# Murmeldyret/cubesat-APDS

Measured on AMD Instinct MI355X. Metric: frames/sec (detect+match+homography) 4k×4k tile vs 1M-desc DB; Mmatches/sec, higher is better.
Workload: dtype fp4 e2m1 operands / f32 accumulate = exact integer Hamming (match), f32 (AKAZE), f64 (homography solve)

## Files before the change

cubesat-apds_amd/csrc/common.h:

```cpp
#pragma once
#include <hip/hip_runtime.h>

#include <atomic>
#include <cstdint>
#include <cstdio>
#include <map>
#include <string>
#include <vector>

#include "../../include/apds.h"

#ifndef APDS_STAGE_WAVE_PRIO
#define APDS_STAGE_WAVE_PRIO 1
#endif
#define APDS_RAISE_WAVE_PRIORITY() __builtin_amdgcn_s_setprio(APDS_STAGE_WAVE_PRIO)

namespace apds {

struct Error {
    int code;
    std::string msg;
};

void set_last_error(const std::string& m);

[[noreturn]] inline void fail(int code, const std::string& m) { throw Error{code, m}; }

inline void hip_check(hipError_t e, const char* what, const char* file, int line) {
    if (e == hipSuccess) return;
    int code = APDS_ERR_INTERNAL;
    if (e == hipErrorNoDevice || e == hipErrorInvalidDevice || e == hipErrorNoBinaryForGpu || e == hipErrorInsufficientDriver ||
        e == hipErrorNotInitialized)
        code = APDS_ERR_NO_DEVICE;
    if (e == hipErrorOutOfMemory) code = APDS_ERR_NOMEM;
    char buf[512];
    snprintf(buf, sizeof buf, "%s failed: %s (%s:%d)", what, hipGetErrorString(e), file, line);
    (void)hipGetLastError();
    throw Error{code, buf};
}
#define HIP_CHECK(x) ::apds::hip_check((x), #x, __FILE__, __LINE__)
#define APDS_REQUIRE(cond, code, msg) \
    do {                               \
        if (!(cond)) ::apds::fail((code), (msg)); \
    } while (0)

struct ThreadCtx {
    int device = 0;
    bool ready = false;
    hipStream_t stream = nullptr;
    std::vector<std::pair<char*, size_t>> slabs;
    size_t slab_used = 0;
    size_t call_bytes = 0;
    bool timing = false;
    struct Ev {
        hipEvent_t a, b;
        hipStream_t s;
    };
    std::map<std::string, std::vector<Ev>> events;
    hipStream_t side = nullptr;
    std::vector<hipEvent_t> fork_events;
    hipEvent_t join_event = nullptr;
    int akaze_first_batch[2] = {8, 8};
    int akaze_batch_streak[2] = {0, 0};
    bool fork_open = false;
    int akaze_kp_estimate = 0;
    int* host_ints = nullptr;
    size_t host_ints_cap = 0;
    int* pinned_ints(size_t n);
    hipStream_t side_stream();
    hipStream_t side_pool[4] = {nullptr, nullptr, nullptr, nullptr};
    hipStream_t side_probe_caller = nullptr, side_probe_choice = nullptr;
    void drop_side();
    hipEvent_t fork_event(size_t i);

    hipEvent_t tail_event = nullptr, count_event = nullptr;
    hipStream_t tail_stream = nullptr;
    bool tail_pending = false;
    void mark_tail(hipStream_t s);
    void mark_tail_noexcept(hipStream_t s) noexcept;

    void ensure();
    void* alloc(size_t bytes);
    void ws_reset(hipStream_t for_stream = nullptr);
    template <class T>
    T* alloc_n(size_t n) { return static_cast<T*>(alloc(n * sizeof(T))); }
};
ThreadCtx& ctx();
std::atomic<int>& live_contexts();

hipStream_t side_stream_beside(hipStream_t caller);
bool take_cached_side_stream(int device, hipStream_t& out);
void cache_side_stream(int device, hipStream_t st);
unsigned stream_event_flags();

inline hipStream_t pick_stream(void* s) { return s ? static_cast<hipStream_t>(s) : ctx().stream; }

struct QueuedWorkspaceCall {
    ThreadCtx& c;
    hipStream_t s;
    explicit QueuedWorkspaceCall(hipStream_t st) : c(ctx()), s(st) { c.ws_reset(s); }
    ~QueuedWorkspaceCall() { c.mark_tail_noexcept(s); }
    QueuedWorkspaceCall(const QueuedWorkspaceCall&) = delete;
    QueuedWorkspaceCall& operator=(const QueuedWorkspaceCall&) = delete;
};

struct KernelTimer {
    ThreadCtx::Ev ev{};
    bool on;
    const char* name;
    KernelTimer(const char* nm, hipStream_t s) : on(ctx().timing), name(nm) {
        if (!on) return;
        ev.s = s;
        HIP_CHECK(hipEventCreate(&ev.a));
        HIP_CHECK(hipEventCreate(&ev.b));
        HIP_CHECK(hipEventRecord(ev.a, s));
    }
    ~KernelTimer() {
        if (!on) return;
        (void)hipEventRecord(ev.b, ev.s);
        ctx().events[name].push_back(ev);
    }
};

struct TraceRange {
    explicit TraceRange(const char* name);
    ~TraceRange();
    TraceRange(const TraceRange&) = delete;
    TraceRange& operator=(const TraceRange&) = delete;
};
#define APDS_RANGE(name) ::apds::TraceRange apds_trace_range_(name)

template <class F>
int guarded(F&& f) {
    try {
        f();
        return APDS_OK;
    } catch (const Error& e) {
        set_last_error(e.msg);
        return e.code;
    } catch (const std::bad_alloc&) {
        set_last_error("host allocation failed");
        return APDS_ERR_NOMEM;
    } catch (const std::exception& e) {
        set_last_error(e.what());
        return APDS_ERR_INTERNAL;
    } catch (...) {
        set_last_error("unknown failure");
        return APDS_ERR_INTERNAL;
    }
}

// ... 12 lines not shown
```

cubesat-apds_amd/csrc/config.h:

```cpp
#pragma once

namespace apds {

struct Config {
    int nld_strip;
    int sf_strip;
    int base_strip;
    int level_strip;
    int level_fuse;
    int level_stream;
    int level_stream_rows;
    int doh_strip;
    int doh_strip_rows;
    int kp_ranked;
    int kp_xcd;
    int half_fuse;
    int fed_shrink;
    int akaze_fork;
    int side_probe;
    int match_mfma;
    int match_mfma_kmax;
    int early_count;
    int l2_prio;
    int match_mfma_lds_pad;
    int match_mfma_prio;
    int match_mfma_sample;
    int match_mfma_splits;
    int match_mfma_xcd;
    int event_scope;
    int debug_host_time;
    int match_lds_cap;
    int match_sample;
    int ransac_batch;
    int pnp_batch;
    int l2_sample_div;
    int pipe_extract_workers;
    int pipe_match_split;
    int pipe_adaptive_cap;
    int pipe_prio;
    int loopback_lag_rank, loopback_lag_ms;
};

const Config& config();

}
```

cubesat-apds_amd/csrc/hamming_mfma.hip:

```cpp
#include <atomic>
#include <memory>

#include "config.h"
#include "kernels.h"
#include "topk_keys.h"

namespace apds {

typedef int hm_v8i __attribute__((ext_vector_type(8)));
typedef float hm_f32x4 __attribute__((ext_vector_type(4)));
typedef uint32_t hm_u32x4 __attribute__((ext_vector_type(4)));

#ifndef APDS_HM_WAVES
#define APDS_HM_WAVES 8
#endif
static constexpr int HM_WAVES = APDS_HM_WAVES;
static constexpr int HM_TM = 16 * HM_WAVES;
#ifndef APDS_HM_WPE
#define APDS_HM_WPE 4
#endif
#ifndef APDS_HM_TOP2_VGPRS
#define APDS_HM_TOP2_VGPRS (APDS_HM_WPE == 4 ? 104 : 512 / APDS_HM_WPE / 8 * 8)
#endif
static_assert(APDS_HM_TOP2_VGPRS % 8 == 0 && APDS_HM_WPE * APDS_HM_TOP2_VGPRS <= 512, "the cap is whole granules that fit the SIMD's file");
// ... 204 lines not shown
__device__ __forceinline__ void hm_load_queries(const uint4* query_fp4, const float* qpc, int nq, int q0, int col, int kq, uint4 (&B)[NC][4], float (&qq)[NC]) {
#pragma unroll
    for (int c = 0; c < NC; c++) {
        const int qi = min(q0 + 16 * c + col, nq - 1);
#pragma unroll
        for (int s = 0; s < 4; s++) B[c][s] = query_fp4[(size_t)qi * 16 + 4 * s + kq];
        qq[c] = qpc[qi];
    }
}
template <bool THR>
__device__ __forceinline__ uint32_t hm_start_value(const uint32_t* thr, int qi) {
    return THR ? thr[qi] : 0x7F800000u;
}
__device__ __forceinline__ uint32_t hm_distance(float qq, uint32_t d) { return (uint32_t)((int)(qq + __uint_as_float(d)) - HM_BIAS); }

template <int PRIO, bool THR>
__global__ __launch_bounds__(64 * HM_WAVES) __attribute__((amdgpu_waves_per_eu(APDS_HM_WPE, APDS_HM_WPE), amdgpu_num_vgpr(APDS_HM_TOP2_VGPRS / 2))) void hamming_mfma_kernel(const uint4* __restrict__ train_fp4, const float* __restrict__ tpc, int n_train,
                                                           const uint4* __restrict__ query_fp4, const float* __restrict__ qpc, int nq, int tiles_per_split,
                                                           int q_tiles, int splits, uint32_t index_base, const uint32_t* __restrict__ thr,
                                                           uint64_t* __restrict__ out) {
    const HmItem w = hm_work_item<HM_NC>(n_train, tiles_per_split, q_tiles, splits);
    const int split = w.split, q0 = w.q0, tile_begin = w.tile_begin, tile_end = w.tile_end, col = w.col, kq = w.kq;
    uint4 B[HM_NC][4];
    hm_load_operands<HM_NC>(query_fp4, nq, q0, col, kq, B);
    HmTop2 best[HM_NC];
#pragma unroll
    for (int c = 0; c < HM_NC; c++) {
        best[c].d0 = hm_start_value<THR>(thr, min(q0 + 16 * c + col, nq - 1));
        hm_settle(best[c].d0);
        best[c].d1 = best[c].d0;
        best[c].i0 = best[c].i1 = 0xFFFFFFFFu;
    }

    if (tile_begin < tile_end) {
        hm_scan_tiles<HM_NC, PRIO>(train_fp4, tpc, tile_begin, tile_end, B, index_base, [&](const hm_f32x4 (&a)[HM_NC], uint32_t row0) {
            bool hit[HM_NC];
#pragma unroll
            for (int c = 0; c < HM_NC; c++) {
                const uint32_t mn = min(min(__float_as_uint(a[c][0]), __float_as_uint(a[c][1])), min(__float_as_uint(a[c][2]), __float_as_uint(a[c][3])));
                hit[c] = mn < best[c].d1;
            }
#pragma unroll
            for (int c = 0; c < HM_NC; c++)
                if (__any(hit[c])) {
#pragma unroll
                    for (int j = 0; j < 4; j++) hm_insert(best[c], __float_as_uint(a[c][j]), row0 + j);
                }
        });
    }
#pragma unroll
    for (int c = 0; c < HM_NC; c++) {
        HmTop2 b = best[c];
#pragma unroll
        for (int off = 16; off < 64; off <<= 1) {
            const uint32_t od0 = (uint32_t)__shfl_xor((int)b.d0, off), od1 = (uint32_t)__shfl_xor((int)b.d1, off);
            const uint32_t oi0 = (uint32_t)__shfl_xor((int)b.i0, off), oi1 = (uint32_t)__shfl_xor((int)b.i1, off);
            HmTop2 m = b;
            auto ins = [&](uint32_t d, uint32_t i) {
                if (i == 0xFFFFFFFFu) return;
                if (d < m.d0 || (d == m.d0 && i < m.i0)) {
                    m.d1 = m.d0;
                    m.i1 = m.i0;
                    m.d0 = d;
                    m.i0 = i;
                } else if ((d < m.d1 || (d == m.d1 && i < m.i1)) && i != m.i0) {
                    m.d1 = d;
                    m.i1 = i;
                }
            };
            ins(od0, oi0);
            ins(od1, oi1);
            b = m;
        }
        const int qi = q0 + 16 * c + col;
        if (kq == 0 && qi < nq) {
            uint64_t* o = out + ((size_t)split * nq + qi) * 2;
            const float qq = qpc[qi];
            o[0] = b.i0 == 0xFFFFFFFFu ? EMPTY_KEY : make_key(hm_distance(qq, b.d0), b.i0);
            o[1] = b.i1 == 0xFFFFFFFFu ? EMPTY_KEY : make_key(hm_distance(qq, b.d1), b.i1);
        }
    }
}

template <int K>
struct HmTopK {
    uint32_t d[K];
    uint32_t i[K];
};
template <int K>
__device__ __forceinline__ void hm_insert_k(HmTopK<K>& b, uint32_t d, uint32_t idx) {
#pragma unroll
    for (int j = K - 1; j > 0; j--) {
        const bool shift = d < b.d[j - 1], here = d < b.d[j];
        b.i[j] = shift ? b.i[j - 1] : (here ? idx : b.i[j]);
        b.d[j] = shift ? b.d[j - 1] : (here ? d : b.d[j]);
    }
    const bool first = d < b.d[0];
    b.i[0] = first ? idx : b.i[0];
    b.d[0] = first ? d : b.d[0];
}
__device__ __forceinline__ uint64_t hm_shfl_xor_u64(uint64_t v, int off) {
    return ((uint64_t)(uint32_t)__shfl_xor((int)(uint32_t)(v >> 32), off) << 32) | (uint32_t)__shfl_xor((int)(uint32_t)v, off);
}

#ifndef APDS_HM_NC_K4
#define APDS_HM_NC_K4 2
#endif
#ifndef APDS_HM_NC_K8
#define APDS_HM_NC_K8 2
#endif
template <int K>
struct HmShape {
    static constexpr int NC = K <= 4 ? APDS_HM_NC_K4 : APDS_HM_NC_K8;
    static constexpr int Q = HM_WAVES * 16 * NC;
};

template <int K, int NC, int PRIO, bool THR>
__global__ __launch_bounds__(64 * HM_WAVES) __attribute__((amdgpu_waves_per_eu(APDS_HM_WPE, APDS_HM_WPE))) void hamming_mfma_topk_kernel(
    const uint4* __restrict__ train_fp4, const float* __restrict__ tpc, int n_train, const uint4* __restrict__ query_fp4, const float* __restrict__ qpc, int nq,
    int tiles_per_split, int q_tiles, int splits, uint32_t index_base, const uint32_t* __restrict__ thr, uint64_t* __restrict__ out) {
    const HmItem w = hm_work_item<NC>(n_train, tiles_per_split, q_tiles, splits);
    const int split = w.split, q0 = w.q0, tile_begin = w.tile_begin, tile_end = w.tile_end, col = w.col, kq = w.kq;
    uint4 B[NC][4];
    float qq[NC];
    hm_load_queries<NC>(query_fp4, qpc, nq, q0, col, kq, B, qq);
    HmTopK<K> best[NC];
#pragma unroll
    for (int c = 0; c < NC; c++) {
        uint32_t start = hm_start_value<THR>(thr, min(q0 + 16 * c + col, nq - 1));
        hm_settle(start), hm_settle(qq[c]);
#pragma unroll
        for (int j = 0; j < K; j++) best[c].d[j] = start, best[c].i[j] = 0xFFFFFFFFu;
    }

    if (tile_begin < tile_end) {
        hm_scan_tiles<NC, PRIO>(train_fp4, tpc, tile_begin, tile_end, B, index_base, [&](const hm_f32x4 (&a)[NC], uint32_t row0) {
            bool hit[NC];
#pragma unroll
            for (int c = 0; c < NC; c++) {
                const uint32_t mn = min(min(__float_as_uint(a[c][0]), __float_as_uint(a[c][1])), min(__float_as_uint(a[c][2]), __float_as_uint(a[c][3])));
                hit[c] = mn < best[c].d[K - 1];
            }
#pragma unroll
            for (int c = 0; c < NC; c++)
                if (__any(hit[c])) {
#pragma unroll
                    for (int j = 0; j < 4; j++) {
                        const uint32_t v = __float_as_uint(a[c][j]);
                        if (__any(v < best[c].d[K - 1])) hm_insert_k<K>(best[c], v, row0 + j);
                    }
                }
        });
    }
#pragma unroll
    for (int c = 0; c < NC; c++) {
        uint64_t key[K];
#pragma unroll
        for (int j = 0; j < K; j++) key[j] = ((uint64_t)best[c].d[j] << 32) | best[c].i[j];
#pragma unroll
        for (int off = 16; off < 64; off <<= 1) {
            uint64_t other[K];
#pragma unroll
            for (int j = 0; j < K; j++) other[j] = hm_shfl_xor_u64(key[j], off);
#pragma unroll
            for (int j = 0; j < K; j++) key[j] = min(key[j], other[K - 1 - j]);
#pragma unroll
            for (int step = K / 2; step > 0; step >>= 1)
#pragma unroll
                for (int j = 0; j < K; j++)
                    if ((j & step) == 0) {
                        const uint64_t lo = min(key[j], key[j + step]), hi = max(key[j], key[j + step]);
                        key[j] = lo;
                        key[j + step] = hi;
                    }
        }
        const int qi = q0 + 16 * c + col;
        if (kq == 0 && qi < nq) {
            uint64_t* o = out + ((size_t)split * nq + qi) * K;
#pragma unroll
            for (int j = 0; j < K; j++) {
                const uint32_t d = key_rank(key[j]), i = key_index(key[j]);
                o[j] = i == 0xFFFFFFFFu ? EMPTY_KEY : make_key(hm_distance(qq[c], d), i);
            }
        }
    }
// ... 22 lines not shown
        for (int sp = 8; sp <= std::min(max_splits, 32); sp += 8) {
            const long long rounds = ceil_div((long long)p.q_tiles * sp, (long long)SLOTS);
            const long long cost = rounds * (ceil_div(t_tiles, sp) + OVERHEAD);
            if (best8 < 0 || cost < best8) best8 = cost, sp8 = sp;
        }
        if (sp8 && best8 * 100 <= best_cost * 105) {
            p.splits = sp8;
            p.tiles_per_split = ceil_div(t_tiles, p.splits);
            return p;
        }
    }
    if (config().match_mfma_splits > 0) p.splits = std::min(t_tiles, config().match_mfma_splits);
    p.tiles_per_split = ceil_div(t_tiles, p.splits);
    p.splits = ceil_div(t_tiles, p.tiles_per_split);
    return p;
}

void hm_expand_device(const void* rows64, long long n, bool query, void* out_fp4, float* pc, hipStream_t s) {
    if (n <= 0) return;
    hipLaunchKernelGGL(hm_expand_rows_kernel, dim3((unsigned)ceil_div(n * 16, 256)), dim3(256), 0, s, static_cast<const uint32_t*>(rows64), n, query ? 0xCu : 0x2u,
                       query ? 0 : HM_BIAS, static_cast<uint4*>(out_fp4), pc);
    if (!query && hm_padded_rows(n) > n)
        hipLaunchKernelGGL(hm_pad_rows_kernel, dim3(1), dim3(128), 0, s, static_cast<uint4*>(out_fp4), pc, n, hm_padded_rows(n));
}
long long hm_padded_rows(long long n) { return ceil_div(n, (long long)HM_TM) * HM_TM; }
long long hm_sample_rows(long long nt) {
    const long long cap = config().match_mfma_sample;
    return (cap > 0 && nt >= 65536) ? std::min<long long>(cap, nt / 16 / HM_TM * HM_TM) / HM_TM * HM_TM : 0;
}

template <class... Kernel>
static void hm_opt_in_lds(std::atomic<bool> (&opted_dev)[64], Kernel... kernel) {
    std::atomic<bool>& opted = opted_dev[ctx().device & 63];
    if (opted.load()) return;
    (HIP_CHECK(hipFuncSetAttribute(reinterpret_cast<const void*>(kernel), hipFuncAttributeMaxDynamicSharedMemorySize, 160 * 1024)), ...);
    opted.store(true);
}

template <int K, class Go>
static void hm_scan_k_launch(Go&& go, bool thr) {
    constexpr int NC = HmShape<K>::NC;
    static std::atomic<bool> opted_dev[64];
    hm_opt_in_lds(opted_dev, &hamming_mfma_topk_kernel<K, NC, 0, false>, &hamming_mfma_topk_kernel<K, NC, 2, false>,
                  &hamming_mfma_topk_kernel<K, NC, 0, true>, &hamming_mfma_topk_kernel<K, NC, 2, true>);
    const bool prio = config().match_mfma_prio > 0;
    if (thr) prio ? go(&hamming_mfma_topk_kernel<K, NC, 2, true>) : go(&hamming_mfma_topk_kernel<K, NC, 0, true>);
    else prio ? go(&hamming_mfma_topk_kernel<K, NC, 2, false>) : go(&hamming_mfma_topk_kernel<K, NC, 0, false>);
}

void hm_scan_device(const void* q_fp4, const float* qpc, int nq, const void* t_fp4, const float* tpc, long long nt, const HmPlan& p, uint32_t index_base,
                    uint64_t* parts, hipStream_t s, const uint32_t* thr, bool timed, int K) {
    APDS_REQUIRE(K <= 2 || K == 4 || K == 8, APDS_ERR_ASSERT, "the matrix-core matcher keeps lists of 2, 4 or 8");
    const size_t lds = (size_t)2 * HM_TM * 256 + 2 * HM_TM * sizeof(float) + (size_t)std::max(0, config().match_mfma_lds_pad);
    auto go = [&](auto kernel) {
        hipLaunchKernelGGL(kernel, dim3((unsigned)p.q_tiles * p.splits), dim3(64 * HM_WAVES), lds, s, static_cast<const uint4*>(t_fp4), tpc, (int)nt,
                           static_cast<const uint4*>(q_fp4), qpc, nq, p.tiles_per_split, p.q_tiles, p.splits, index_base, thr, parts);
    };
    std::unique_ptr<KernelTimer> timer, timer_k;
    if (timed) timer.reset(new KernelTimer("hamming_topk", s));
    if (timed && K > 2) timer_k.reset(new KernelTimer("hamming_topk_mfma_k", s));
    if (K == 4) return hm_scan_k_launch<4>(go, thr != nullptr);
    if (K == 8) return hm_scan_k_launch<8>(go, thr != nullptr);
    static std::atomic<bool> opted_dev[64];
    hm_opt_in_lds(opted_dev, &hamming_mfma_kernel<0, false>, &hamming_mfma_kernel<1, false>, &hamming_mfma_kernel<2, false>, &hamming_mfma_kernel<3, false>,
                  &hamming_mfma_kernel<0, true>, &hamming_mfma_kernel<1, true>, &hamming_mfma_kernel<2, true>, &hamming_mfma_kernel<3, true>);
    const int prio = std::max(0, std::min(3, config().match_mfma_prio));
    if (thr) {
        switch (prio) {
            case 0: go(&hamming_mfma_kernel<0, true>); break;
            case 1: go(&hamming_mfma_kernel<1, true>); break;
            case 2: go(&hamming_mfma_kernel<2, true>); break;
            default: go(&hamming_mfma_kernel<3, true>); break;
        }
    } else {
        switch (prio) {
            case 0: go(&hamming_mfma_kernel<0, false>); break;
            case 1: go(&hamming_mfma_kernel<1, false>); break;
            case 2: go(&hamming_mfma_kernel<2, false>); break;
            default: go(&hamming_mfma_kernel<3, false>); break;
        }
    }
}

void* hm_train_create(const void* rows64, long long n, hipStream_t s) {
    APDS_REQUIRE(rows64 && n > 0 && n < (1ll << 31), APDS_ERR_ASSERT, "an expanded train set needs rows");
    HmTrain* t = new HmTrain();
    t->device = ctx().device;
    t->src = rows64;
    t->n = n;
    if (hipMalloc(&t->rows, (size_t)hm_padded_rows(n) * 256) != hipSuccess || hipMalloc(reinterpret_cast<void**>(&t->pc), (size_t)hm_padded_rows(n) * 4) != hipSuccess) {
        (void)hipGetLastError();
        if (t->rows) (void)hipFree(t->rows);
        delete t;
        fail(APDS_ERR_NOMEM, "no device memory for the expanded train rows");
    }
    hm_expand_device(rows64, n, false, t->rows, t->pc, s);
    HIP_CHECK(hipStreamSynchronize(s));
    return t;
}
void hm_train_destroy(void* h) {
    HmTrain* t = static_cast<HmTrain*>(h);
    if (!t) return;
    int previous = -1;
    if (hipGetDevice(&previous) != hipSuccess) previous = -1;
    (void)hipSetDevice(t->device);
    (void)hipDeviceSynchronize();
    if (t->rows) (void)hipFree(t->rows);
    if (t->pc) (void)hipFree(t->pc);
    delete t;
    if (previous >= 0) (void)hipSetDevice(previous);
}

static void hm_topk_expanded(const void* q, int nq, const void* t4, const float* tp, long long nt, uint32_t index_base, int k, uint64_t* out, hipStream_t s) {
    ThreadCtx& c = ctx();
    void* q4 = c.alloc((size_t)nq * 256);
    float* qp = c.alloc_n<float>(nq);
    {
        KernelTimer timer("hamming_topk_sample", s);
        hm_expand_device(q, nq, true, q4, qp, s);
    }
    const long long sample = hm_sample_rows(nt);
    const int K = hm_list_len(k);
    uint64_t* topk = k == K ? out : c.alloc_n<uint64_t>((size_t)nq * K);
    const HmPlan p = hm_plan(nq, nt - sample, K);
    const int lists = p.splits + (sample ? 1 : 0);
    uint64_t* parts = lists == 1 ? topk : c.alloc_n<uint64_t>((size_t)lists * nq * K);
    uint32_t* thr = nullptr;
    if (sample) {
        const HmPlan pa = hm_plan(nq, sample, K);
        uint64_t* parts_a = c.alloc_n<uint64_t>((size_t)pa.splits * nq * K);
        uint64_t* topk_a = parts + (size_t)p.splits * nq * K;
        thr = c.alloc_n<uint32_t>(nq);
        KernelTimer timer("hamming_topk_sample", s);
        hm_scan_device(q4, qp, nq, t4, tp, sample, pa, index_base, parts_a, s, nullptr, false, K);
        if (pa.splits > 1) merge_topk_device(parts_a, pa.splits, nq, K, topk_a, s);
        else HIP_CHECK(hipMemcpyAsync(topk_a, parts_a, (size_t)nq * K * 8, hipMemcpyDeviceToDevice, s));
        hipLaunchKernelGGL(hm_thresholds_kernel, dim3(ceil_div(nq, 256)), dim3(256), 0, s, (const uint64_t*)topk_a, K, (const float*)qp, nq, thr);
    }
    hm_scan_device(q4, qp, nq, static_cast<const char*>(t4) + (size_t)sample * 256, tp + sample, nt - sample, p, index_base + (uint32_t)sample, parts, s, thr,
                   true, K);
    if (lists > 1) merge_topk_device(parts, lists, nq, K, topk, s);
    if (k != K) take_first_columns_device(topk, nq, K, k, out, s);
    HIP_CHECK(hipGetLastError());
}

void hamming_mfma_topk_device(const void* q, int nq, const void* t, long long nt, uint32_t index_base, int k, uint64_t* out, hipStream_t s) {
    APDS_REQUIRE(k >= 1 && k <= 8, APDS_ERR_ASSERT, "the matrix-core matcher serves 1 <= k <= 8");
    APDS_REQUIRE(nq > 0 && nt > 0 && nt < (1ll << 31), APDS_ERR_ASSERT, "the matrix-core matcher needs queries and train rows");
    ThreadCtx& c = ctx();
    void* t4 = c.alloc((size_t)hm_padded_rows(nt) * 256);
    float* tp = c.alloc_n<float>(hm_padded_rows(nt));
    {
        KernelTimer timer("hamming_topk_sample", s);
        hm_expand_device(t, nt, false, t4, tp, s);
    }
    hm_topk_expanded(q, nq, t4, tp, nt, index_base, k, out, s);
}

void hamming_mfma_topk_train_device(const void* q, int nq, const void* train, uint32_t index_base, int k, uint64_t* out, hipStream_t s) {
    const HmTrain* t = static_cast<const HmTrain*>(train);
    APDS_REQUIRE(t && k >= 1 && k <= 8 && nq > 0, APDS_ERR_ASSERT, "the matrix-core matcher needs an expanded train set, queries and 1 <= k <= 8");
    hm_topk_expanded(q, nq, t->rows, t->pc, t->n, index_base, k, out, s);
}

__global__ void hm_plain_popcounts_kernel(const float* __restrict__ biased, long long n, float* __restrict__ plain) {
    const long long i = (long long)blockIdx.x * blockDim.x + threadIdx.x;
    if (i < n) plain[i] = biased[i] - (float)HM_BIAS;
}

void hm_train_plain_popcounts_device(const void* train, float* out, hipStream_t s) {
    const HmTrain* t = static_cast<const HmTrain*>(train);
    APDS_REQUIRE(t && out, APDS_ERR_ASSERT, "an expanded train set and an output are required");
    hipLaunchKernelGGL(hm_plain_popcounts_kernel, dim3((unsigned)ceil_div(t->n, 256ll)), dim3(256), 0, s, (const float*)t->pc, (long long)t->n, out);
    HIP_CHECK(hipGetLastError());
}

void hamming_mfma_swapped_top1_device(const void* rows64, int n, const void* train, const float* train_plain_pc, uint64_t* train_best, hipStream_t s) {
    const HmTrain* t = static_cast<const HmTrain*>(train);
    APDS_REQUIRE(t && train_plain_pc && rows64 && train_best && n > 0, APDS_ERR_ASSERT, "the swapped scan needs an expanded train set, its plain popcounts and rows");
    ThreadCtx& c = ctx();
    const long long n_pad = hm_padded_rows(n);
    uint4* f4 = static_cast<uint4*>(c.alloc((size_t)n_pad * 256));
    float* fp = c.alloc_n<float>((size_t)n_pad);
    {
        KernelTimer timer("hamming_topk_sample", s);
        hipLaunchKernelGGL(hm_expand_rows_kernel, dim3((unsigned)ceil_div((long long)n * 16, 256ll)), dim3(256), 0, s, static_cast<const uint32_t*>(rows64), (long long)n, 0xCu,
                           HM_BIAS, f4, fp);
        if (n_pad > n) hipLaunchKernelGGL(hm_pad_rows_kernel, dim3(1), dim3(128), 0, s, f4, fp, (long long)n, n_pad);
    }
    const int nc = (int)t->n;
    const HmPlan p = hm_plan(nc, n, 2);
    uint64_t* top2 = c.alloc_n<uint64_t>((size_t)nc * 2);
    uint64_t* parts = p.splits == 1 ? top2 : c.alloc_n<uint64_t>((size_t)p.splits * nc * 2);
    hm_scan_device(t->rows, train_plain_pc, nc, f4, fp, n, p, 0, parts, s, nullptr, true, 2);
    if (p.splits > 1) merge_topk_device(parts, p.splits, nc, 2, top2, s);
    take_first_columns_device(top2, nc, 2, 1, train_best, s);
    HIP_CHECK(hipGetLastError());
}

}
```

cubesat-apds_amd/csrc/pipeline.cpp:

```cpp
#include <chrono>
#include <climits>
#include <cmath>
#include <condition_variable>
#include <cstring>
#include <deque>
#include <map>
#include <memory>
#include <mutex>
#include <thread>

#include "config.h"
#include "kernels.h"

using namespace apds;

namespace {

template <class T>
class Chan {
    std::mutex m;
    std::condition_variable cv;
    std::deque<T> q;
    bool closed = false;

// ... 168 lines not shown
            fail(e.code, std::string(what) + ": " + e.msg);
        } catch (const std::exception& e) {
            fail(APDS_ERR_INTERNAL, std::string(what) + ": " + e.what());
        }
        (void)apds_dev_timing_enable(0);
        (void)apds_thread_release();
    }

    void finish(Slot* s, const apds_frame_result& r, const std::string& why, const apds_frame_pose* fp = nullptr) {
        {
            std::lock_guard<std::mutex> g(m);
            results[s->index] = r;
            if (fp) poses[s->index] = *fp;
            if (r.status != APDS_OK) result_errors[s->index] = why;
            done++;
        }
        cv.notify_all();
        q_free[(size_t)s->owner]->push(s);
    }

    void extract_worker(int e) {
        hipStream_t st = st_extract[e];
        Slot* s = nullptr;
        while (q_jobs[(size_t)e]->pop(s)) {
            if (!s) {
                harvest({"akaze_extract"});
                continue;
            }
            const void* img = s->src;
            s->status = APDS_OK;
            s->K = 0;
            if (!s->on_device) {
                const size_t bytes = s->stride * (size_t)p.rows;
                if (s->frame_dev_bytes < bytes) {
                    if (s->frame_dev) HIP_CHECK(hipFree(s->frame_dev));
                    s->frame_dev = nullptr;
                    HIP_CHECK(hipMalloc(reinterpret_cast<void**>(&s->frame_dev), bytes));
                    s->frame_dev_bytes = bytes;
                }
                HIP_CHECK(hipMemcpyAsync(s->frame_dev, s->src, bytes, hipMemcpyHostToDevice, st));
                img = s->frame_dev;
            }
            int n = 0;
            const int rc = apds_dev_akaze_extract(img, p.rows, p.cols, p.channels, s->stride, cap, s->kps, s->desc, cap, &n, st);
            if (rc != APDS_OK) {
                s->status = rc;
                s->error = apds_last_error();
                n = 0;
            }
            s->K = n;
            HIP_CHECK(hipEventRecord(s->ev_extract, st));
            if (extract_delay_s > 0) std::this_thread::sleep_for(std::chrono::duration<double>(extract_delay_s));
            q_ext[(size_t)e]->push(s);
            if (world == 1) q_any.push(e);
        }
        collect({"akaze_extract"});
    }

    void match_worker() {
        bool watch = adaptive_cap;
        if (p.match_lds_cap > 0) set_thread_scan_cap(p.match_lds_cap), watch = false;
        std::deque<std::pair<Slot*, Slot*>> pending;
        std::vector<float> recent;
        Slot* prev = nullptr;
        int e = 0;
        int64_t seen = 0;
        while (q_any.pop(e)) {
            const bool crosscheck = matcher == APDS_PIPELINE_MATCH_CROSSCHECK;
            if (e < 0) {
                harvest({"hamming_topk", "hamming_topk_sample"});
                continue;
            }
            Slot* s = nullptr;
            if (!q_ext[(size_t)e]->pop(s)) break;
            const int K = s->K;
            if (table) {
                s->n_view = 0;
                PIPE_OK(apds_db_view_select(s->view, s->sel.mode, s->sel.value, s->sel.x_start, s->sel.y_start, s->sel.x_end, s->sel.y_end, pose_on ? 1 : 0,
                                            st_match, &s->n_view));
                void* xyz = nullptr;
                PIPE_OK(apds_db_view_pointers(s->view, nullptr, nullptr, nullptr, nullptr, &xyz, nullptr));
                s->view_xyz = xyz;
                HIP_CHECK(hipStreamWaitEvent(st_match, s->ev_extract, 0));
                HIP_CHECK(hipEventRecord(s->ev_mstart, st_match));
                if (s->n_view < 2) {
                    if (s->status == APDS_OK) {
                        s->status = APDS_ERR_ASSERT;
                        s->error = "the frame's selection has fewer than two rows: a train set of at least two rows is required";
                    }
                } else if (K > 0 && crosscheck) {
                    PIPE_OK(apds_dev_hamming_topk(s->view_rows64, s->n_view, s->desc, K, 0, 1, s->train_best, st_match));
                } else if (K > 0) {
                    PIPE_OK(apds_dev_hamming_topk(s->desc, K, s->view_rows64, s->n_view, 0, 2, s->keys, st_match));
                }
                HIP_CHECK(hipEventRecord(s->ev_match, st_match));
                HIP_CHECK(hipEventRecord(s->ev_mend, st_match));
            } else if (K > 0 && split && !crosscheck) {
                HIP_CHECK(hipStreamWaitEvent(st_pre, s->ev_extract, 0));
                PIPE_OK(apds_dev_topk_prepass(s->topk_state, s->desc, K, db_rows, n_rows, index_base, 2, st_pre));
                HIP_CHECK(hipEventRecord(s->ev_pre, st_pre));
                HIP_CHECK(hipStreamWaitEvent(st_match, s->ev_pre, 0));
                HIP_CHECK(hipEventRecord(s->ev_mstart, st_match));
                PIPE_OK(apds_dev_topk_scan(s->topk_state, s->desc, db_rows, st_match));
                HIP_CHECK(hipEventRecord(s->ev_scan, st_match));
                HIP_CHECK(hipEventRecord(s->ev_mend, st_match));
                HIP_CHECK(hipStreamWaitEvent(st_merge, s->ev_scan, 0));
                PIPE_OK(apds_dev_topk_merge(s->topk_state, index_base, s->keys, st_merge));
                HIP_CHECK(hipEventRecord(s->ev_match, st_merge));
            } else {
                HIP_CHECK(hipStreamWaitEvent(st_match, s->ev_extract, 0));
                HIP_CHECK(hipEventRecord(s->ev_mstart, st_match));
                if (K > 0 && crosscheck && db_expanded) {
                    PIPE_OK(guarded([&] {
                        QueuedWorkspaceCall call(st_match);
                        hamming_mfma_swapped_top1_device(s->desc, K, db_expanded, db_plain_pc, s->train_best, st_match);
                    }));
                } else if (K > 0 && crosscheck) {
                    PIPE_OK(apds_dev_hamming_topk(db_rows, (int)n_rows, s->desc, K, 0, 1, s->train_best, st_match));
                } else if (K > 0 && db_expanded) {
                    PIPE_OK(guarded([&] {
                        QueuedWorkspaceCall call(st_match);
                        hamming_mfma_topk_train_device(s->desc, K, db_expanded, index_base, 2, static_cast<uint64_t*>(s->keys), st_match);
                    }));
                } else if (K > 0) {
                    PIPE_OK(apds_dev_hamming_topk(s->desc, K, db_rows, n_rows, index_base, 2, s->keys, st_match));
                }
                HIP_CHECK(hipEventRecord(s->ev_match, st_match));
                HIP_CHECK(hipEventRecord(s->ev_mend, st_match));
            }
            if (watch && !crosscheck) {
                if (prev && seen >= 4) pending.emplace_back(prev, s);
                while (!pending.empty() && hipEventQuery(pending.front().second->ev_mstart) == hipSuccess) {
                    float g = -1;
                    if (hipEventElapsedTime(&g, pending.front().first->ev_mend, pending.front().second->ev_mstart) != hipSuccess) (void)hipGetLastError(), g = -1;
                    pending.pop_front();
                    if (g >= 0 && g < 1000) {
                        recent.push_back(g);
                        std::lock_guard<std::mutex> lk(m);
                        gaps.push_back(g);
                    }
                }
                (void)hipGetLastError();
                int late = 0;
                for (size_t i = recent.size() >= 6 ? recent.size() - 6 : 0; i < recent.size(); i++) late += recent[i] > 4.0f;
                if (recent.size() >= 6 && late >= 3 && cap_bytes == 0) {
                    set_thread_scan_cap(55000);
                    std::lock_guard<std::mutex> lk(m);
                    cap_bytes = 55000;
                    cap_frame = (int)s->index;
                    for (size_t i = recent.size() - 6; i < recent.size(); i++) cap_gaps.push_back(recent[i]);
                    watch = false;
                }
            }
            prev = s;
            seen++;
            q_homography.push(s);
        }
        collect({"hamming_topk", "hamming_topk_sample"});
        q_homography.close();
    }

    void sharded_match_worker() {
        constexpr int NEXT_FLAG = 1 << 30;
        Slot* prev = nullptr;
        for (int64_t i = 0;; i++) {
            Slot* s = nullptr;
            if (!q_ext[(size_t)(i % E)]->pop(s)) break;
            if (!s) {
                harvest({"hamming_topk", "hamming_topk_sample"});
                i--;
                continue;
            }
            bool next_here;
            {
                std::lock_guard<std::mutex> g(m);
                next_here = next_submit > i + 1;
            }
            s->counts.assign((size_t)world, 0);
            PIPE_OK(apds_shard_counts(shard, s->K | (next_here ? NEXT_FLAG : 0), s->counts.data(), st_counts));
            bool next_everywhere = true;
            for (int& c : s->counts) {
                next_everywhere = next_everywhere && (c & NEXT_FLAG);
                c &= NEXT_FLAG - 1;
            }
            HIP_CHECK(hipStreamWaitEvent(st_gather, s->ev_extract, 0));
            PIPE_OK(apds_shard_gather(shard, s->shard_slot, s->K ? s->desc : nullptr, s->K, s->counts.data(), st_gather));
            auto finish_exchange = [&](Slot* f) {
                PIPE_OK(apds_shard_exchange_merge(shard, f->shard_slot, 2, f->keys, st_match));
                HIP_CHECK(hipEventRecord(f->ev_match, st_match));
                q_homography.push(f);
            };
            if (prev) finish_exchange(prev);
            prev = nullptr;
            PIPE_OK(apds_shard_scan(shard, s->shard_slot, 2, st_match));
            if (next_everywhere) prev = s;
            else finish_exchange(s);
        }
        collect({"hamming_topk", "hamming_topk_sample"});
        q_homography.close();
    }

    void homography_worker() {
        hipStream_t st = st_homography;
        Slot* s = nullptr;
        int* count_dev = nullptr;
        HIP_CHECK(hipMalloc(reinterpret_cast<void**>(&count_dev), 256));
        while (q_homography.pop(s)) {
            if (!s) {
                harvest({"ransac_score"});
                continue;
            }
// ... 474 lines not shown
```

cubesat-apds_amd/csrc/runtime.cpp:

```cpp
#include <chrono>
#include <dlfcn.h>
#include <cstdlib>
#include <cstring>

#include <mutex>
#include <vector>

#include <atomic>

#include "common.h"
#include "config.h"

namespace apds {

const Config& config() {
    static const Config c = [] {
        auto env = [](const char* name, int dflt) {
            const char* v = getenv(name);
            return v && *v ? atoi(v) : dflt;
        };
        Config k;
        k.nld_strip = env("APDS_NLD_STRIP", 1);
        k.sf_strip = env("APDS_SF_STRIP", 1);
        k.base_strip = env("APDS_BASE_STRIP", 1);
        k.level_strip = env("APDS_LEVEL_STRIP", 1);
        k.level_fuse = env("APDS_LEVEL_FUSE", 1);
        k.level_stream = env("APDS_LEVEL_STREAM", 1);
        k.level_stream_rows = env("APDS_LEVEL_STREAM_ROWS", 0);
        k.doh_strip = env("APDS_DOH_STRIP", 1);
        k.doh_strip_rows = env("APDS_DOH_STRIP_ROWS", 0);
        k.kp_ranked = env("APDS_KP_RANKED", 1);
        k.kp_xcd = env("APDS_KP_XCD", 1);
        k.fed_shrink = env("APDS_FED_SHRINK", 1);
        k.half_fuse = env("APDS_HALF_FUSE", 1);
        k.akaze_fork = env("APDS_AKAZE_FORK", 1);
        k.side_probe = env("APDS_SIDE_PROBE", 1);
        k.event_scope = env("APDS_EVENT_SCOPE", 2);
        k.match_mfma = env("APDS_MATCH_MFMA", 1);
        k.match_mfma_kmax = std::max(2, std::min(8, env("APDS_MATCH_MFMA_KMAX", 8)));
        k.match_mfma_xcd = env("APDS_MATCH_MFMA_XCD", 1);
        k.match_mfma_splits = env("APDS_MATCH_MFMA_SPLITS", 0);
        k.match_mfma_sample = env("APDS_MATCH_MFMA_SAMPLE", 16384);
        k.match_mfma_prio = env("APDS_MATCH_MFMA_PRIO", 2);
        k.l2_prio = env("APDS_L2_PRIO", 1);
        k.early_count = env("APDS_EARLY_COUNT", 1);
        k.match_mfma_lds_pad = env("APDS_MATCH_MFMA_LDS_PAD", 0);
        k.debug_host_time = env("APDS_DEBUG_HOST_TIME", 0);
        k.match_lds_cap = env("APDS_MATCH_LDS_CAP", 0);
        k.match_sample = env("APDS_MATCH_SAMPLE", 16384);
        k.ransac_batch = env("APDS_RANSAC_BATCH", 512);
        k.pnp_batch = env("APDS_PNP_BATCH", 2048);
        k.l2_sample_div = std::max(1, env("APDS_L2_SAMPLE_DIV", 12));
        k.pipe_extract_workers = std::max(1, env("APDS_EXTRACT_WORKERS", 2));
        k.pipe_match_split = env("APDS_MATCH_SPLIT", 1);
        k.pipe_adaptive_cap = env("APDS_ADAPTIVE_CAP", 1);
        k.pipe_prio = env("APDS_PIPE_PRIO", -1);
        k.loopback_lag_rank = -1;
        k.loopback_lag_ms = 0;
        if (const char* lag = getenv("APDS_TEST_LOOPBACK_LAG")) {
            int r = -1, ms = 0;
            if (sscanf(lag, "%d:%d", &r, &ms) == 2 && r >= 0 && ms > 0) k.loopback_lag_rank = r, k.loopback_lag_ms = ms;
        }
        return k;
    }();
    return c;
}

namespace {
struct Roctx {
    int (*push)(const char*) = nullptr;
    int (*pop)() = nullptr;
    Roctx() {
        for (const char* lib : {"librocprofiler-sdk-roctx.so", "librocprofiler-sdk-roctx.so.1", "libroctx64.so", "libroctx64.so.4"}) {
            void* h = dlopen(lib, RTLD_LAZY | RTLD_LOCAL);
            if (!h) continue;
            push = reinterpret_cast<int (*)(const char*)>(dlsym(h, "roctxRangePushA"));
            pop = reinterpret_cast<int (*)()>(dlsym(h, "roctxRangePop"));
            if (push && pop) return;
            push = nullptr;
            pop = nullptr;
        }
    }
};
const Roctx& roctx() {
    static const Roctx r;
    return r;
}
}
TraceRange::TraceRange(const char* name) {
    if (roctx().push) roctx().push(name);
}
TraceRange::~TraceRange() {
    if (roctx().pop) roctx().pop();
}

static thread_local std::string g_last_error;
static thread_local ThreadCtx g_ctx;

void set_last_error(const std::string& m) { g_last_error = m; }
ThreadCtx& ctx() {
    g_ctx.ensure();
    return g_ctx;
}

void ThreadCtx::ensure() {
    if (ready) return;
    int n = 0;
    hipError_t e = hipGetDeviceCount(&n);
    if (e != hipSuccess || n <= 0) {
        (void)hipGetLastError();
        fail(APDS_ERR_NO_DEVICE, "no HIP device available: libapds_hip has no CPU fallback");
    }
    if (device >= n) fail(APDS_ERR_NO_DEVICE, "device ordinal out of range");
    HIP_CHECK(hipSetDevice(device));
    HIP_CHECK(hipStreamCreateWithFlags(&stream, hipStreamNonBlocking));
    ready = true;
    live_contexts().fetch_add(1);
}

std::atomic<int>& live_contexts() {
    static std::atomic<int> n{0};
    return n;
}

hipStream_t ThreadCtx::side_stream() {
    if (!side) {
        HIP_CHECK(hipStreamCreateWithPriority(&side, hipStreamNonBlocking, 0));
    }
    return side;
}

namespace {
std::mutex g_side_cache_mutex;
std::vector<std::pair<int, hipStream_t>> g_side_cache;
}
bool take_cached_side_stream(int device, hipStream_t& out) {
    std::lock_guard<std::mutex> g(g_side_cache_mutex);
    for (size_t i = 0; i < g_side_cache.size(); i++)
        if (g_side_cache[i].first == device) {
            out = g_side_cache[i].second;
            g_side_cache.erase(g_side_cache.begin() + i);
            return true;
        }
    return false;
}
void cache_side_stream(int device, hipStream_t st) {
    std::lock_guard<std::mutex> g(g_side_cache_mutex);
    g_side_cache.emplace_back(device, st);
}

int* ThreadCtx::pinned_ints(size_t n) {
    if (n > host_ints_cap) {
        if (host_ints) (void)hipHostFree(host_ints);
        host_ints = nullptr;
        host_ints_cap = 0;
        const size_t cap = std::max<size_t>(64, n * 2);
        HIP_CHECK(hipHostMalloc(reinterpret_cast<void**>(&host_ints), cap * sizeof(int), hipHostMallocDefault));
        host_ints_cap = cap;
    }
    return host_ints;
}

void ThreadCtx::drop_side() {
    if (host_ints) (void)hipHostFree(host_ints);
    host_ints = nullptr;
    host_ints_cap = 0;
    side_probe_caller = side_probe_choice = nullptr;
    for (hipStream_t& st : side_pool)
        if (st) {
            (void)hipStreamSynchronize(st);
            cache_side_stream(device, st);
            st = nullptr;
        }
    if (side) {
        (void)hipStreamSynchronize(side);
        (void)hipStreamDestroy(side);
        side = nullptr;
    }
    for (hipEvent_t e : fork_events) (void)hipEventDestroy(e);
    fork_events.clear();
    if (join_event) (void)hipEventDestroy(join_event);
    join_event = nullptr;
    fork_open = false;
    if (tail_event) (void)hipEventSynchronize(tail_event), (void)hipEventDestroy(tail_event);
    if (count_event) (void)hipEventDestroy(count_event);
    tail_event = count_event = nullptr;
    tail_pending = false;
}

unsigned stream_event_flags() {
    const int scope = config().event_scope;
    return hipEventDisableTiming | (scope == 2 ? (unsigned)hipEventDisableSystemFence : scope == 0 ? (unsigned)hipEventReleaseToDevice : 0u);
}

hipEvent_t ThreadCtx::fork_event(size_t i) {
    while (fork_events.size() <= i) {
        hipEvent_t e = nullptr;
        HIP_CHECK(hipEventCreateWithFlags(&e, stream_event_flags()));
        fork_events.push_back(e);
    }
    return fork_events[i];
}

namespace {
struct SlabCache {
    std::mutex m;
    std::vector<std::pair<int, std::pair<char*, size_t>>> free;
};
SlabCache& slab_cache() {
    static SlabCache c;
    return c;
}
bool take_cached_slab(int device, size_t want, std::pair<char*, size_t>& out) {
    SlabCache& c = slab_cache();
    std::lock_guard<std::mutex> g(c.m);
    int best = -1;
    for (int i = 0; i < (int)c.free.size(); i++)
        if (c.free[i].first == device && c.free[i].second.second >= want && (best < 0 || c.free[i].second.second > c.free[best].second.second)) best = i;
    if (best < 0) return false;
    out = c.free[best].second;
    c.free.erase(c.free.begin() + best);
    return true;
}
void cache_slab(int device, std::pair<char*, size_t> s) {
    SlabCache& c = slab_cache();
    std::lock_guard<std::mutex> g(c.m);
    c.free.emplace_back(device, s);
}
}

void* ThreadCtx::alloc(size_t bytes) {
    bytes = (bytes + 255) & ~size_t(255);
    if (bytes == 0) bytes = 256;
    call_bytes += bytes;
    if (slabs.empty() || slab_used + bytes > slabs.back().second) {
        const size_t want = std::max(bytes + bytes / 8, size_t(1) << 24);
        std::pair<char*, size_t> got;
        if (take_cached_slab(device, want, got)) {
            slabs.push_back(got);
        } else {
            char* p = nullptr;
            HIP_CHECK(hipMalloc(&p, want));
            slabs.emplace_back(p, want);
        }
        slab_used = 0;
    }
    void* r = slabs.back().first + slab_used;
    slab_used += bytes;
    return r;
// ... 218 lines not shown
```

Before: 153.5.

## Fuse sample top-2 scan, split merge and threshold computation into one kernel

For the K=2 sampled prepass, a new kernel scans the sample rows and does an in-wave top-2 reduction. The last-arriving block per query tile, found with an atomic arrival counter, merges the split partials and writes thresholds. This replaces the separate scan, merge/memcpy and threshold launches, and also stops recording match start/end events when the watch flag is off. It adds cross-block atomics and fences plus a persistent counter buffer that must reset correctly between calls.

```diff
diff --git a/cubesat-apds_amd/csrc/common.h b/cubesat-apds_amd/csrc/common.h
--- a/cubesat-apds_amd/csrc/common.h
+++ b/cubesat-apds_amd/csrc/common.h
@@ -67,6 +67,9 @@
     int* host_ints = nullptr;
     size_t host_ints_cap = 0;
     int* pinned_ints(size_t n);
+    uint32_t* arrive = nullptr;
+    size_t arrive_cap = 0;
+    uint32_t* arrival_counters(size_t n, hipStream_t s);
     hipStream_t side_stream();
     hipStream_t side_pool[4] = {nullptr, nullptr, nullptr, nullptr};
     hipStream_t side_probe_caller = nullptr, side_probe_choice = nullptr;
diff --git a/cubesat-apds_amd/csrc/config.h b/cubesat-apds_amd/csrc/config.h
--- a/cubesat-apds_amd/csrc/config.h
+++ b/cubesat-apds_amd/csrc/config.h
@@ -25,6 +25,8 @@
     int match_mfma_lds_pad;
     int match_mfma_prio;
     int match_mfma_sample;
+    int match_mfma_fused_thr;
+    int match_mfma_sample_splits;
     int match_mfma_splits;
     int match_mfma_xcd;
     int event_scope;
diff --git a/cubesat-apds_amd/csrc/hamming_mfma.hip b/cubesat-apds_amd/csrc/hamming_mfma.hip
--- a/cubesat-apds_amd/csrc/hamming_mfma.hip
+++ b/cubesat-apds_amd/csrc/hamming_mfma.hip
@@ -310,6 +310,90 @@
     }
 }
 
+__device__ __forceinline__ uint64_t hm_shfl_xor_u64(uint64_t v, int off) {
+    return ((uint64_t)(uint32_t)__shfl_xor((int)(uint32_t)(v >> 32), off) << 32) | (uint32_t)__shfl_xor((int)(uint32_t)v, off);
+}
+
+template <int PRIO>
+__global__ __launch_bounds__(64 * HM_WAVES) __attribute__((amdgpu_waves_per_eu(APDS_HM_WPE, APDS_HM_WPE), amdgpu_num_vgpr(APDS_HM_TOP2_VGPRS / 2))) void hm_threshold_scan_kernel(
+    const uint4* __restrict__ train_fp4, const float* __restrict__ tpc, int n_train, const uint4* __restrict__ query_fp4, const float* __restrict__ qpc, int nq,
+    int tiles_per_split, int q_tiles, int splits, uint32_t index_base, uint64_t* parts, uint64_t* __restrict__ topk, uint32_t* __restrict__ thr,
+    uint32_t* __restrict__ arrive) {
+    {
+        const HmItem w = hm_work_item<HM_NC>(n_train, tiles_per_split, q_tiles, splits);
+        const int split = w.split, q0 = w.q0, tile_begin = w.tile_begin, tile_end = w.tile_end, col = w.col, kq = w.kq;
+        uint4 B[HM_NC][4];
+        hm_load_operands<HM_NC>(query_fp4, nq, q0, col, kq, B);
+        HmTop2 best[HM_NC];
+#pragma unroll
+        for (int c = 0; c < HM_NC; c++) {
+            best[c].d0 = hm_start_value<false>(nullptr, 0);
+            hm_settle(best[c].d0);
+            best[c].d1 = best[c].d0;
+            best[c].i0 = best[c].i1 = 0xFFFFFFFFu;
+        }
+        if (tile_begin < tile_end) {
+            hm_scan_tiles<HM_NC, PRIO>(train_fp4, tpc, tile_begin, tile_end, B, index_base, [&](const hm_f32x4 (&a)[HM_NC], uint32_t row0) {
+                bool hit[HM_NC];
+#pragma unroll
+                for (int c = 0; c < HM_NC; c++) {
+                    const uint32_t mn = min(min(__float_as_uint(a[c][0]), __float_as_uint(a[c][1])), min(__float_as_uint(a[c][2]), __float_as_uint(a[c][3])));
+                    hit[c] = mn < best[c].d1;
+                }
+#pragma unroll
+                for (int c = 0; c < HM_NC; c++)
+                    if (__any(hit[c])) {
+#pragma unroll
+                        for (int j = 0; j < 4; j++) hm_insert(best[c], __float_as_uint(a[c][j]), row0 + j);
+                    }
+            });
+        }
+#pragma unroll
+        for (int c = 0; c < HM_NC; c++) {
+            uint64_t k0 = ((uint64_t)best[c].d0 << 32) | best[c].i0, k1 = ((uint64_t)best[c].d1 << 32) | best[c].i1;
+#pragma unroll
+            for (int off = 16; off < 64; off <<= 1) {
+                const uint64_t o0 = hm_shfl_xor_u64(k0, off), o1 = hm_shfl_xor_u64(k1, off);
+                const uint64_t lo = min(k0, o0);
+                k1 = min(max(k0, o0), min(k1, o1));
+                k0 = lo;
+            }
+            const int qi = q0 + 16 * c + col;
+            if (kq == 0 && qi < nq) {
+                uint64_t* o = parts + ((size_t)split * nq + qi) * 2;
+                const float qq = qpc[qi];
+                o[0] = key_index(k0) == 0xFFFFFFFFu ? EMPTY_KEY : make_key(hm_distance(qq, key_rank(k0)), key_index(k0));
+                o[1] = key_index(k1) == 0xFFFFFFFFu ? EMPTY_KEY : make_key(hm_distance(qq, key_rank(k1)), key_index(k1));
+            }
+        }
+    }
+    extern __shared__ __attribute__((aligned(128))) unsigned char hm_lds[];
+    uint32_t* arrived = reinterpret_cast<uint32_t*>(hm_lds);
+    const int qtile = ((splits & 7) == 0 ? (int)(blockIdx.x >> 3) : (int)blockIdx.x) % q_tiles;
+    hm_dma_wait();
+    __syncthreads();
+    if (threadIdx.x == 0) {
+        __builtin_amdgcn_fence(__ATOMIC_RELEASE, "agent");
+        *arrived = atomicAdd(&arrive[qtile], 1u);
+    }
+    __syncthreads();
+    if (*arrived != (uint32_t)splits - 1) return;
+    __builtin_amdgcn_fence(__ATOMIC_ACQUIRE, "agent");
+    if (threadIdx.x == 0) arrive[qtile] = 0;
+    const int qi = qtile * HM_Q + (int)threadIdx.x;
+    if ((int)threadIdx.x >= HM_Q || qi >= nq) return;
+    uint64_t best[2] = {EMPTY_KEY, EMPTY_KEY};
+    for (int p = 0; p < splits; p++) {
+        const uint64_t* src = parts + ((size_t)p * nq + qi) * 2;
+        const uint64_t k0 = __hip_atomic_load(src, __ATOMIC_RELAXED, __HIP_MEMORY_SCOPE_AGENT), k1 = __hip_atomic_load(src + 1, __ATOMIC_RELAXED, __HIP_MEMORY_SCOPE_AGENT);
+        topk_insert<2>(best, k0);
+        topk_insert<2>(best, k1);
+    }
+    topk[(size_t)qi * 2] = best[0];
+    topk[(size_t)qi * 2 + 1] = best[1];
+    thr[qi] = best[1] == EMPTY_KEY ? 0x7F800000u : __float_as_uint((float)((int)key_rank(best[1]) - (int)qpc[qi] + HM_BIAS));
+}
+
 template <int K>
 struct HmTopK {
     uint32_t d[K];
@@ -326,9 +410,6 @@
     const bool first = d < b.d[0];
     b.i[0] = first ? idx : b.i[0];
     b.d[0] = first ? d : b.d[0];
-}
-__device__ __forceinline__ uint64_t hm_shfl_xor_u64(uint64_t v, int off) {
-    return ((uint64_t)(uint32_t)__shfl_xor((int)(uint32_t)(v >> 32), off) << 32) | (uint32_t)__shfl_xor((int)(uint32_t)v, off);
 }
 
 #ifndef APDS_HM_NC_K4
@@ -517,6 +598,24 @@
     }
 }
 
+static void hm_threshold_scan_device(const void* q_fp4, const float* qpc, int nq, const void* t_fp4, const float* tpc, long long nt, const HmPlan& p,
+                                     uint32_t index_base, uint64_t* parts, uint64_t* topk, uint32_t* thr, hipStream_t s) {
+    const size_t lds = (size_t)2 * HM_TM * 256 + 2 * HM_TM * sizeof(float) + (size_t)std::max(0, config().match_mfma_lds_pad);
+    uint32_t* arrive = ctx().arrival_counters((size_t)p.q_tiles, s);
+    auto go = [&](auto kernel) {
+        hipLaunchKernelGGL(kernel, dim3((unsigned)p.q_tiles * p.splits), dim3(64 * HM_WAVES), lds, s, static_cast<const uint4*>(t_fp4), tpc, (int)nt,
+                           static_cast<const uint4*>(q_fp4), qpc, nq, p.tiles_per_split, p.q_tiles, p.splits, index_base, parts, topk, thr, arrive);
+    };
+    static std::atomic<bool> opted_dev[64];
+    hm_opt_in_lds(opted_dev, &hm_threshold_scan_kernel<0>, &hm_threshold_scan_kernel<1>, &hm_threshold_scan_kernel<2>, &hm_threshold_scan_kernel<3>);
+    switch (std::max(0, std::min(3, config().match_mfma_prio))) {
+        case 0: go(&hm_threshold_scan_kernel<0>); break;
+        case 1: go(&hm_threshold_scan_kernel<1>); break;
+        case 2: go(&hm_threshold_scan_kernel<2>); break;
+        default: go(&hm_threshold_scan_kernel<3>); break;
+    }
+}
+
 void* hm_train_create(const void* rows64, long long n, hipStream_t s) {
     APDS_REQUIRE(rows64 && n > 0 && n < (1ll << 31), APDS_ERR_ASSERT, "an expanded train set needs rows");
     HmTrain* t = new HmTrain();
@@ -550,10 +649,8 @@
     ThreadCtx& c = ctx();
     void* q4 = c.alloc((size_t)nq * 256);
     float* qp = c.alloc_n<float>(nq);
-    {
-        KernelTimer timer("hamming_topk_sample", s);
-        hm_expand_device(q, nq, true, q4, qp, s);
-    }
+    std::unique_ptr<KernelTimer> front(new KernelTimer("hamming_topk_sample", s));
+    hm_expand_device(q, nq, true, q4, qp, s);
     const long long sample = hm_sample_rows(nt);
     const int K = hm_list_len(k);
     uint64_t* topk = k == K ? out : c.alloc_n<uint64_t>((size_t)nq * K);
@@ -562,16 +659,25 @@
     uint64_t* parts = lists == 1 ? topk : c.alloc_n<uint64_t>((size_t)lists * nq * K);
     uint32_t* thr = nullptr;
     if (sample) {
-        const HmPlan pa = hm_plan(nq, sample, K);
+        HmPlan pa = hm_plan(nq, sample, K);
+        if (config().match_mfma_sample_splits > 0) {
+            const int t_tiles = (int)(sample / HM_TM);
+            pa.tiles_per_split = ceil_div(t_tiles, std::min(t_tiles, config().match_mfma_sample_splits));
+            pa.splits = ceil_div(t_tiles, pa.tiles_per_split);
+        }
         uint64_t* parts_a = c.alloc_n<uint64_t>((size_t)pa.splits * nq * K);
         uint64_t* topk_a = parts + (size_t)p.splits * nq * K;
         thr = c.alloc_n<uint32_t>(nq);
-        KernelTimer timer("hamming_topk_sample", s);
-        hm_scan_device(q4, qp, nq, t4, tp, sample, pa, index_base, parts_a, s, nullptr, false, K);
-        if (pa.splits > 1) merge_topk_device(parts_a, pa.splits, nq, K, topk_a, s);
-        else HIP_CHECK(hipMemcpyAsync(topk_a, parts_a, (size_t)nq * K * 8, hipMemcpyDeviceToDevice, s));
-        hipLaunchKernelGGL(hm_thresholds_kernel, dim3(ceil_div(nq, 256)), dim3(256), 0, s, (const uint64_t*)topk_a, K, (const float*)qp, nq, thr);
-    }
+        if (K == 2 && config().match_mfma_fused_thr) {
+            hm_threshold_scan_device(q4, qp, nq, t4, tp, sample, pa, index_base, parts_a, topk_a, thr, s);
+        } else {
+            hm_scan_device(q4, qp, nq, t4, tp, sample, pa, index_base, parts_a, s, nullptr, false, K);
+            if (pa.splits > 1) merge_topk_device(parts_a, pa.splits, nq, K, topk_a, s);
+            else HIP_CHECK(hipMemcpyAsync(topk_a, parts_a, (size_t)nq * K * 8, hipMemcpyDeviceToDevice, s));
+            hipLaunchKernelGGL(hm_thresholds_kernel, dim3(ceil_div(nq, 256)), dim3(256), 0, s, (const uint64_t*)topk_a, K, (const float*)qp, nq, thr);
+        }
+    }
+    front.reset();
     hm_scan_device(q4, qp, nq, static_cast<const char*>(t4) + (size_t)sample * 256, tp + sample, nt - sample, p, index_base + (uint32_t)sample, parts, s, thr,
                    true, K);
     if (lists > 1) merge_topk_device(parts, lists, nq, K, topk, s);
diff --git a/cubesat-apds_amd/csrc/pipeline.cpp b/cubesat-apds_amd/csrc/pipeline.cpp
--- a/cubesat-apds_amd/csrc/pipeline.cpp
+++ b/cubesat-apds_amd/csrc/pipeline.cpp
@@ -274,7 +274,7 @@
                 PIPE_OK(apds_db_view_pointers(s->view, nullptr, nullptr, nullptr, nullptr, &xyz, nullptr));
                 s->view_xyz = xyz;
                 HIP_CHECK(hipStreamWaitEvent(st_match, s->ev_extract, 0));
-                HIP_CHECK(hipEventRecord(s->ev_mstart, st_match));
+                if (watch) HIP_CHECK(hipEventRecord(s->ev_mstart, st_match));
                 if (s->n_view < 2) {
                     if (s->status == APDS_OK) {
                         s->status = APDS_ERR_ASSERT;
@@ -286,22 +286,22 @@
                     PIPE_OK(apds_dev_hamming_topk(s->desc, K, s->view_rows64, s->n_view, 0, 2, s->keys, st_match));
                 }
                 HIP_CHECK(hipEventRecord(s->ev_match, st_match));
-                HIP_CHECK(hipEventRecord(s->ev_mend, st_match));
+                if (watch) HIP_CHECK(hipEventRecord(s->ev_mend, st_match));
             } else if (K > 0 && split && !crosscheck) {
                 HIP_CHECK(hipStreamWaitEvent(st_pre, s->ev_extract, 0));
                 PIPE_OK(apds_dev_topk_prepass(s->topk_state, s->desc, K, db_rows, n_rows, index_base, 2, st_pre));
                 HIP_CHECK(hipEventRecord(s->ev_pre, st_pre));
                 HIP_CHECK(hipStreamWaitEvent(st_match, s->ev_pre, 0));
-                HIP_CHECK(hipEventRecord(s->ev_mstart, st_match));
+                if (watch) HIP_CHECK(hipEventRecord(s->ev_mstart, st_match));
                 PIPE_OK(apds_dev_topk_scan(s->topk_state, s->desc, db_rows, st_match));
                 HIP_CHECK(hipEventRecord(s->ev_scan, st_match));
-                HIP_CHECK(hipEventRecord(s->ev_mend, st_match));
+                if (watch) HIP_CHECK(hipEventRecord(s->ev_mend, st_match));
                 HIP_CHECK(hipStreamWaitEvent(st_merge, s->ev_scan, 0));
                 PIPE_OK(apds_dev_topk_merge(s->topk_state, index_base, s->keys, st_merge));
                 HIP_CHECK(hipEventRecord(s->ev_match, st_merge));
             } else {
                 HIP_CHECK(hipStreamWaitEvent(st_match, s->ev_extract, 0));
-                HIP_CHECK(hipEventRecord(s->ev_mstart, st_match));
+                if (watch) HIP_CHECK(hipEventRecord(s->ev_mstart, st_match));
                 if (K > 0 && crosscheck && db_expanded) {
                     PIPE_OK(guarded([&] {
                         QueuedWorkspaceCall call(st_match);
@@ -318,7 +318,7 @@
                     PIPE_OK(apds_dev_hamming_topk(s->desc, K, db_rows, n_rows, index_base, 2, s->keys, st_match));
                 }
                 HIP_CHECK(hipEventRecord(s->ev_match, st_match));
-                HIP_CHECK(hipEventRecord(s->ev_mend, st_match));
+                if (watch) HIP_CHECK(hipEventRecord(s->ev_mend, st_match));
             }
             if (watch && !crosscheck) {
                 if (prev && seen >= 4) pending.emplace_back(prev, s);
diff --git a/cubesat-apds_amd/csrc/runtime.cpp b/cubesat-apds_amd/csrc/runtime.cpp
--- a/cubesat-apds_amd/csrc/runtime.cpp
+++ b/cubesat-apds_amd/csrc/runtime.cpp
@@ -41,6 +41,8 @@
         k.match_mfma_xcd = env("APDS_MATCH_MFMA_XCD", 1);
         k.match_mfma_splits = env("APDS_MATCH_MFMA_SPLITS", 0);
         k.match_mfma_sample = env("APDS_MATCH_MFMA_SAMPLE", 16384);
+        k.match_mfma_fused_thr = env("APDS_MATCH_MFMA_FUSED_THR", 1);
+        k.match_mfma_sample_splits = env("APDS_MATCH_MFMA_SAMPLE_SPLITS", 0);
         k.match_mfma_prio = env("APDS_MATCH_MFMA_PRIO", 2);
         k.l2_prio = env("APDS_L2_PRIO", 1);
         k.early_count = env("APDS_EARLY_COUNT", 1);
@@ -161,10 +163,26 @@
     return host_ints;
 }
 
+uint32_t* ThreadCtx::arrival_counters(size_t n, hipStream_t s) {
+    if (n > arrive_cap) {
+        if (arrive) HIP_CHECK(hipFree(arrive));
+        arrive = nullptr;
+        arrive_cap = 0;
+        const size_t cap = std::max<size_t>(1024, n * 2);
+        HIP_CHECK(hipMalloc(reinterpret_cast<void**>(&arrive), cap * sizeof(uint32_t)));
+        arrive_cap = cap;
+        HIP_CHECK(hipMemsetAsync(arrive, 0, cap * sizeof(uint32_t), s));
+    }
+    return arrive;
+}
+
 void ThreadCtx::drop_side() {
     if (host_ints) (void)hipHostFree(host_ints);
     host_ints = nullptr;
     host_ints_cap = 0;
+    if (arrive) (void)hipFree(arrive);
+    arrive = nullptr;
+    arrive_cap = 0;
     side_probe_caller = side_probe_choice = nullptr;
     for (hipStream_t& st : side_pool)
         if (st) {
```

Result: no change. 152.9 (-0.4%).
